# sharonct/CTPA-CLIP

Hardware: AMD Instinct MI355X
Metric: CT-report pairs/sec (contrastive step) (higher is better)
Workload: dtype bf16

## Files before the change

ctpa-clip_amd/csrc/gemm.hip:

```cpp
#include <algorithm>
#include "common.h"
#include "../../include/ctclip_hip.h"

int ctclip_gemm256(const ctclip_gemm_args* a, int split, int batch, void* stream);

namespace {

constexpr int BM = 128, BN = 128, BKT = 64, NTH = 256;
constexpr int KROW = BKT * 2 + 16;
constexpr int TILE_BYTES = 128 * KROW;
constexpr int SMEM_BYTES = 4 * TILE_BYTES;
constexpr int CS_LD = 132;

struct P {
  int64_t M, N, K;
  const u16* A; int64_t lda;
  const u16* B; int64_t ldb;
  const u16* B2;
  void* C; int64_t ldc; int c_f32;
  u16* C2; int64_t ldc2;
  const float* bias;
  const void* R; int64_t ldr; int r_f32;
  float alpha; int act; int accumulate; int split_k;
  int64_t sA, sB, sC, sC2, sR;
// ... 647 lines not shown
    hipLaunchKernelGGL(reduce_slabs_rows_kernel<false>, dim3(blocks), dim3(256), 0, (hipStream_t)stream, slabs, nslab,
                       rows, cols, ld, map, dst, ldd, accumulate);
  CT_CHECK_LAUNCH();
  return 0;
}

extern "C" int ctclip_reduce_slabs(const float* slabs, int64_t nslab, int64_t rows, int64_t cols, int64_t ld,
                                   void* out, int64_t ldo, int32_t out_f32, int32_t accumulate, void* stream) {
  if (rows == 0 || cols == 0) return 0;
  CT_REQUIRE(cols % 4 == 0 && ld % 4 == 0 && ldo % 4 == 0, CT_EALIGN);
  const int64_t total = rows * (cols / 4);
  if (total < 64 * 1024 && nslab >= 16) {
    hipLaunchKernelGGL(reduce_slabs_skinny_kernel, dim3(cdiv(total, 64)), dim3(1024), 0, (hipStream_t)stream, slabs,
                       nslab, rows, cols, ld, out, ldo, out_f32, accumulate);
    CT_CHECK_LAUNCH();
    return 0;
  }
  const int blocks = (int)std::min<int64_t>(4096, (total + 255) / 256);
  hipLaunchKernelGGL(reduce_slabs_kernel, dim3(blocks), dim3(256), 0, (hipStream_t)stream, slabs, nslab, rows, cols,
                     ld, out, ldo, out_f32, accumulate);
  CT_CHECK_LAUNCH();
  return 0;
}
```

ctpa-clip_amd/ctclip_mi355x/_lib.py:

```python
from __future__ import annotations

import ctypes
import os

import torch

_HERE = os.path.dirname(os.path.abspath(__file__))
LIB_PATH = os.environ.get('CTCLIP_HIP_LIB') or os.path.join(_HERE, 'libctclip_hip.so')
_LIB = None

c_i64 = ctypes.c_int64
c_i32 = ctypes.c_int32
c_f32 = ctypes.c_float
c_vp = ctypes.c_void_p


class SlabJob(ctypes.Structure):
    _fields_ = [('slabs', c_vp), ('nslab', c_i64), ('cols', c_i64), ('out', c_vp), ('accumulate', c_i32),
                ('pad', c_i32)]


ABI_VERSION = 2


class GemmArgs(ctypes.Structure):
    _fields_ = [
        ('M', c_i64), ('N', c_i64), ('K', c_i64),
        ('A', c_vp), ('lda', c_i64), ('a_kcontig', c_i32),
        ('B', c_vp), ('ldb', c_i64), ('b_kcontig', c_i32),
        ('C', c_vp), ('ldc', c_i64), ('c_f32', c_i32),
        ('C2', c_vp), ('ldc2', c_i64),
        ('bias', c_vp),
        ('R', c_vp), ('ldr', c_i64), ('r_f32', c_i32),
        ('alpha', c_f32),
        ('act', c_i32),
        ('accumulate', c_i32),
        ('split_k', c_i32),
        ('batch', c_i32),
        ('sA', c_i64), ('sB', c_i64), ('sC', c_i64), ('sC2', c_i64), ('sR', c_i64),
        ('n2', c_i32),
        ('B2', c_vp),
        ('ab_f16', c_i32),
        ('r_f16', c_i32),
# ... 157 lines not shown
    'ctclip_gemm_set_grid_cap': [c_i32],
    'ctclip_reduce_slabs_ep': [c_vp, c_i64, c_i64, c_i64, c_i64, ctypes.POINTER(GemmArgs), c_vp],
    'ctclip_reduce_slabs_ep_drop': [c_vp, c_i64, c_i64, c_i64, c_i64, ctypes.POINTER(GemmArgs), c_f32, ctypes.c_uint64,
                                    c_vp],
    'ctclip_layernorm_bwd_drop': [c_vp, c_i32, c_i64, c_vp, c_i32, c_i64, c_vp, c_vp, c_vp, c_i64, c_i32, c_vp, c_i64,
                                  c_vp, c_i64, c_vp, c_vp, c_vp, c_i32, c_f32, ctypes.c_uint64, c_vp],
    'ctclip_patch_ln_x2': [c_vp, c_i32, c_i32, c_i64, c_i32, c_i32, c_i32, c_i32, c_i32, c_i32, c_vp, c_f32, c_vp,
                           c_vp, c_i64, c_vp],
    'ctclip_patch_ln_x3': [c_vp, c_i32, c_i32, c_i64, c_i32, c_i32, c_i32, c_i32, c_i32, c_i32, c_vp, c_f32, c_vp,
                           c_vp, c_vp, c_i64, c_vp],
    'ctclip_layernorm_fwd_x2': [c_vp, c_i32, c_i64, c_i64, c_i32, c_vp, c_vp, c_f32, c_vp, c_vp, c_i64, c_vp, c_i64,
                                c_vp, c_vp, c_vp],
    'ctclip_layernorm_fwd_x3': [c_vp, c_i32, c_i64, c_i64, c_i32, c_vp, c_vp, c_f32, c_vp, c_vp, c_vp, c_i64, c_vp,
                                c_i64, c_vp, c_vp, c_vp, c_vp],
    'ctclip_pack_rows_h16': [c_vp, c_i64, c_vp, c_i64, c_i32, c_i32, c_vp, c_vp, c_i64, c_vp],
    'ctclip_pack_qkv_fold_h16': [c_vp, c_i64, c_vp, c_i64, c_i64, c_vp, c_i64, c_i64, c_vp, c_i64, c_vp, c_vp],
    'ctclip_skinny_gemm_slices': [c_i64, c_i64, c_i64],
    'ctclip_skinny_gemm': [c_vp, c_i64, c_vp, c_i64, c_i64, c_i64, c_i64, c_vp, c_i32, c_vp],
    'ctclip_vq_l2norm_h16': [c_vp, c_i64, c_i64, c_i32, c_vp, c_i64, c_vp],
    'ctclip_skinny_sgemm_slices': [c_i64, c_i64, c_i64],
    'ctclip_skinny_sgemm': [c_vp, c_i64, c_vp, c_i64, c_i64, c_i64, c_i64, c_vp, c_i32, c_vp],
    'ctclip_reduce_slabs': [c_vp, c_i64, c_i64, c_i64, c_i64, c_vp, c_i64, c_i32, c_i32, c_vp],
    'ctclip_reduce_slabs_multi': [ctypes.POINTER(SlabJob), c_i32, c_vp],
    'ctclip_layernorm_fwd': [c_vp, c_i32, c_i64, c_i64, c_i32, c_vp, c_vp, c_f32, c_vp, c_i64, c_vp, c_i64,
                             c_vp, c_vp, c_vp],
    'ctclip_layernorm_bwd': [c_vp, c_i32, c_i64, c_vp, c_i32, c_i64, c_vp, c_vp, c_vp, c_i64, c_i32, c_vp, c_i64,
                             c_vp, c_i64, c_vp, c_i64, c_vp, c_vp, c_i32, c_vp],
    'ctclip_l2norm_scale_fwd': [c_vp, c_i64, c_i64, c_i32, c_i32, c_vp, c_vp, c_i64, c_vp],
    'ctclip_l2norm_scale_bwd': [c_vp, c_i64, c_vp, c_i64, c_i64, c_i32, c_i32, c_vp, c_vp, c_i64, c_vp, c_i32, c_vp],
    'ctclip_l2norm_scale_bwd_fold': [c_vp, c_i64, c_vp, c_i64, c_i64, c_i32, c_i32, c_vp, c_vp, c_i64, c_vp, c_i32,
                                     c_vp, c_vp, c_vp, c_i64, c_vp, c_vp, c_i32, c_vp, c_vp, c_vp],
    'ctclip_colsum': [c_vp, c_i32, c_i64, c_i64, c_i32, c_vp, c_i32, c_vp],
    'ctclip_geglu_bwd': [c_vp, c_i64, c_vp, c_i64, c_i64, c_i32, c_vp, c_i64, c_vp],
    'ctclip_gelu_bwd': [c_vp, c_vp, c_vp, c_i64, c_vp],
    'ctclip_pack_rows': [c_vp, c_i64, c_vp, c_i64, c_i32, c_i32, c_vp, c_vp, c_i64, c_vp],
    'ctclip_pack_rows_f32': [c_vp, c_i64, c_vp, c_i64, c_i32, c_i32, c_vp, c_vp, c_i64, c_vp],
    'ctclip_split_f16': [c_vp, c_i64, c_i64, c_i32, c_f32, c_vp, c_vp, c_i64, c_vp, c_vp],
    'ctclip_pack_rows_x3': [c_vp, c_i64, c_vp, c_i64, c_i32, c_i32, c_vp, c_f32, c_vp, c_vp, c_i64, c_vp, c_vp],
    'ctclip_sgemm_tn': [ctypes.POINTER(SgemmTnArgs), c_vp],
    'ctclip_unpack_rows': [c_vp, c_i64, c_vp, c_i64, c_i32, c_vp, c_i64, c_i32, c_vp],
    'ctclip_reduce_slabs_rows': [c_vp, c_i64, c_i64, c_i64, c_i64, c_vp, c_vp, c_i64, c_i32, c_vp],
    'ctclip_gelu_f32': [c_vp, c_vp, c_i64, c_vp],
    'ctclip_cast_f32_bf16': [c_vp, c_vp, c_i64, c_vp],
    'ctclip_cast_f32_bf16_split': [c_vp, c_vp, c_vp, c_i64, c_vp],
    'ctclip_add_f32': [c_vp, c_vp, c_vp, c_vp, c_i64, c_vp],
    'ctclip_patch_ln': [c_vp, c_i32, c_i32, c_i64, c_i32, c_i32, c_i32, c_i32, c_i32, c_i32, c_vp, c_f32, c_vp, c_i64,
# ... 128 lines not shown
```

ctpa-clip_amd/ctclip_mi355x/functional.py:

```python
from __future__ import annotations

import math
import os
import weakref
from dataclasses import dataclass

import torch

from . import dist_sync
from . import kernels as K
from . import streams

F32, BF16 = torch.float32, torch.bfloat16


def gsink(p):
    if not p.requires_grad:
        return None
    if p.grad is None:
        p.grad = torch.zeros_like(p, memory_format=torch.contiguous_format)
    return p.grad


def gsink_cat(ps):
# ... 521 lines not shown
            x3f = K.linear(g, W2p, residual=x2f, out_dtype=F32, out2=x3b)
        else:
            h = K.linear(xn2, W1p, act=K.ACT_GEGLU, out2=g, tag='ff1',
                         flops=2.0 * xf.shape[0] * W1.shape[0] * W1.shape[1])
            x3f = K.linear(g, W2p, residual=x2f, out_dtype=F32, out2=x3b)
        if lean:
            ctx.mark_non_differentiable(x3b)
            return x3f, x3b
        ctx.geo = geo
        ctx.use_bias = use_bias
        ctx.fold = fold
        ctx.fold_w = (Wp, cs) if fold else None
        ctx.params = (peg_w, peg_b, norm_g, q_scale, k_scale, Wq, Wkv, Wo, ff_w, ff_b, W1, W2)
        ctx.save_for_backward(xb, x1b, m1, r1, xn, q, kv, qn, kn, o, lse, x2b, m2, r2, xn2, h, g,
                              bias_u if use_bias else torch.empty(0), Wq_b, Wkv_b, Wo_b, W1p, W2p)
        ctx.mark_non_differentiable(x3b)
        ctx.set_materialize_grads(False)
        return x3f, x3b

    @staticmethod
    def backward(ctx, dx3f, _dx3b):
        if dx3f is None:
            return (None,) * 16
        (xb, x1b, m1, r1, xn, q, kv, qn, kn, o, lse, x2b, m2, r2, xn2, h, g, bias_u, Wq_b, Wkv_b, Wo_b, W1p,
         W2p) = ctx.saved_tensors
        peg_w, peg_b, norm_g, q_scale, k_scale, Wq, Wkv, Wo, ff_w, ff_b, W1, W2 = ctx.params
        geo = ctx.geo
        H, dh = geo.heads, geo.dim_head
        inner = H * dh
        dev = dx3f.device
        dx3b = take_shadow(dx3f)
        dx3f = dx3f.contiguous()
        if dx3b is None:
            dx3b = K.cast_bf16(dx3f)
        dh_ = K.matmul_nn_geglu_bwd(dx3b, W2p, h)
        M_ = dx3b.shape[0]
        if gsink(W2) is not None:
            K.matmul_tn(dx3b, g, tag='dw', flops=2.0 * M_ * W2.shape[0] * W2.shape[1],
                        unpack=(gsink(W2), None, W2.shape[1]))
        fused = K.matmul_nn_ln_bwd(dh_, W1p, x2b, m2, r2, ff_w, dx3f, dgamma_out=gsink(ff_w),
                                   dbeta_out=gsink(ff_b)) if K.ln_guarded() else None
        if fused is None:
            dxn2 = K.matmul_nn(dh_, W1p)
        if gsink(W1) is not None:
            rmap = ff1_rowmap(W1.shape[0] // 2, dev)
            K.matmul_tn(dh_, xn2, tag='dw', flops=2.0 * M_ * W1.shape[0] * W1.shape[1],
                        unpack=(gsink(W1), rmap, W1.shape[1]))
        if fused is not None:
            dx2f, dx2b = fused
        else:
            dx2f, dx2b, _, _ = K.layernorm_bwd(dxn2, x2b, m2, r2, ff_w, dres=dx3f, dgamma_out=gsink(ff_w),
                                               dbeta_out=gsink(ff_b))
        do = K.matmul_nn(dx2b, Wo_b)
        K.matmul_tn(dx2b, o, out=gsink(Wo), accumulate=True, tag='dw')
        dqn = torch.empty_like(qn)
        dkn = torch.empty_like(kn)
        L, nseq, seq = geo.seq()
        du = None
        if ctx.use_bias:
            acc = ctx.bias_acc
            if acc['du'] is None:
                acc['du'] = torch.zeros_like(bias_u)
            du = acc['du']
        fold = getattr(ctx, 'fold', False)
        if fold:
            Wp, cs = ctx.fold_w
            M_ = qn.shape[0]
            dqkv = torch.empty(M_, 3 * inner, device=dev, dtype=BF16)
            dqkn = torch.empty(M_, 2 * inner, device=dev, dtype=BF16)
            K.attn_bwd(qn, kn, kv[:, inner:], o, lse, do, dqkn[:, :inner], dqkn[:, inner:], dqkv[:, 2 * inner:],
                       L=L, H=H, D=dh, nseq=nseq, scale=8.0, seq=seq, bias_u=bias_u if ctx.use_bias else None,
                       dbias_u=du, grid=(geo.Hg, geo.Wg) if ctx.use_bias else (0, 0))
            _bias_grad_ready(ctx, du)
            qk = q.as_strided((M_, 2 * inner), q.stride())
            _, _, u1, c1, be1 = K.l2norm_qk_bwd_fold(qk, dqkn, q_scale, k_scale, r1, m1, dqkv[:, :2 * inner], cs,
                                                     x1b.shape[1], ds_q_out=gsink(q_scale),
                                                     ds_k_out=gsink(k_scale))
            Gqkv = K.matmul_tn(dqkv, x1b, tag='dw')
            gq, gkv = gsink(Wq), gsink(Wkv)
            K.lnfold_wgrad(Gqkv, u1, norm_g, gq if gq is not None else torch.empty(Wq.shape, device=dev),
                           wq=Wq.detach(), grad_gamma=gsink(norm_g),
                           grad_rest=gkv if gkv is not None else torch.empty(Wkv.shape, device=dev))
            dx1f, dx1b = K.matmul_lnfold_bwd(dqkv, Wp, dx2f, x1b, c1, be1)
        else:
            dkv = torch.empty_like(kv)
            K.attn_bwd(qn, kn, kv[:, inner:], o, lse, do, dqn, dkn, dkv[:, inner:], L=L, H=H, D=dh, nseq=nseq,
                       scale=8.0, seq=seq, bias_u=bias_u if ctx.use_bias else None, dbias_u=du,
                       grid=(geo.Hg, geo.Wg) if ctx.use_bias else (0, 0))
            _bias_grad_ready(ctx, du)
            dq = torch.empty(q.shape, device=dev, dtype=q.dtype)
            K.l2norm_scale_bwd(q, dqn, H, dh, q_scale, dq, ds_out=gsink(q_scale))
            K.l2norm_scale_bwd(kv[:, :inner], dkn, H, dh, k_scale, dkv[:, :inner], ds_out=gsink(k_scale))
            fusable = K.ln_guarded() and K.ln_fusable(dq.shape[0], Wq_b.shape[1], bwd=True)
            if not fusable:
                dxn = K.matmul_nn(dq, Wq_b)
            K.matmul_tn(dq, xn, out=gsink(Wq), accumulate=True, tag='dw')
            K.matmul_tn(dkv, x1b, out=gsink(Wkv), accumulate=True, tag='dw')
            dx1kv = K.matmul_nn(dkv, Wkv_b, residual=dx2f, out_dtype=F32)
            fused = K.matmul_nn_ln_bwd(dq, Wq_b, x1b, m1, r1, norm_g, dx1kv, dgamma_out=gsink(norm_g)) \
                if fusable else None
            if fused is not None:
                dx1f, dx1b = fused
            else:
                if fusable:
                    dxn = K.matmul_nn(dq, Wq_b)
                dx1f, dx1b, _, _ = K.layernorm_bwd(dxn, x1b, m1, r1, norm_g, dres=dx1kv, want_beta=False,
                                                   dgamma_out=gsink(norm_g))
        dxf, dxb, _, _ = K.peg_bwd(dx1b, dx1f, xb, geo.B, geo.T, geo.Hg, geo.Wg, peg_w, geo.mode,
                                   dweight_out=gsink(peg_w), dbias_out=gsink(peg_b))
        put_shadow(dxf, dxb)
        if du is not None:
            if ctx.bias_first:
                ctx.bias_acc['du'] = None
            else:
                du = None
        return (dxf, None, du, None, None, None, None, None, None, None, None, None, None,
                None, None, None)


def _fold_shape_ok(geo, dim, Wkv):
# ... 596 lines not shown
```

ctpa-clip_amd/ctclip_mi355x/kernels.py:

```python
from __future__ import annotations

import contextlib
import os

import torch

from . import _lib
from ._lib import GemmArgs, LnEpilogueArgs, call, ptr, stream_ptr

BF16 = torch.bfloat16
F32 = torch.float32
F16 = torch.float16

ACT_NONE, ACT_GELU, ACT_GEGLU, ACT_ARGMAX, ACT_GEGLU_BWD, ACT_L2N, ACT_GELU_BWD = 0, 1, 2, 3, 4, 5, 6


def _chk(t, name, dtype=None):
    if not t.is_cuda:
        raise ValueError(f'{name}: expected a device tensor')
    if dtype is not None and t.dtype != dtype:
        raise ValueError(f'{name}: expected {dtype}, got {t.dtype}')


class KernelTimer:
# ... 276 lines not shown
    reduce_param_partials(pg, dgamma_out, True)
    if dbeta_out is not None:
        reduce_param_partials(pb, dbeta_out, True)
    return dxf, dxb


def matmul_nn_gelu_bwd(dy, w, pre, out=None):
    M, N = dy.shape
    K = w.shape[1]
    assert w.shape[0] == N and pre.shape == (M, K) and pre.dtype == BF16
    if out is None:
        out = torch.empty(M, K, device=dy.device, dtype=BF16)
    gemm_raw(M, K, N, dy, dy.stride(0), True, w, w.stride(0), False, out, out.stride(0), R=pre, ldr=pre.stride(0),
             act=ACT_GELU_BWD)
    return out


def split_for(m_rows, tiles):
    target = 512
    s = max(1, min(target // max(tiles, 1), m_rows // 1024))
    return max(1, s)


def matmul_tn(dy, x, *, out=None, accumulate=False, split_k=None, alpha=1.0, tag=None, flops=None, unpack=None):
    M, N = dy.shape
    K = x.shape[1]
    assert x.shape[0] == M
    if out is None:
        out = torch.zeros(N, K, device=dy.device, dtype=F32) if accumulate else \
            torch.empty(N, K, device=dy.device, dtype=F32)
    if split_k is not None:
        s = split_k
    elif N >= 256 and K >= 256 and M % 64 == 0 and M >= 64 * 1024:
        t256 = ((N + 255) // 256) * ((K + 255) // 256)
        s = max(1, 256 // t256)
        if t256 * s < 160:
            s = split_for(M, ((N + 127) // 128) * ((K + 127) // 128))
    else:
        s = split_for(M, ((N + 127) // 128) * ((K + 127) // 128))
    if s <= 1:
        gemm_raw(N, K, M, dy, dy.stride(0), False, x, x.stride(0), False, out, out.stride(0),
                 accumulate=accumulate, alpha=alpha, tag=tag, flops=flops)
        if unpack is not None:
            dst, rowmap, cols = unpack
            return unpack_rows(out, dst, rowmap=rowmap, cols=cols, accumulate=True)
        return out
    slabs = torch.empty(s, N, K, device=dy.device, dtype=F32)
    gemm_raw(N, K, M, dy, dy.stride(0), False, x, x.stride(0), False, slabs, K, split_k=s, alpha=alpha, tag=tag,
             flops=flops)
    if unpack is not None:
        dst, rowmap, cols = unpack
        assert dst.dtype == F32 and dst.stride(1) == 1 and cols <= K
        assert rowmap is None or (rowmap.dtype == torch.int32 and rowmap.numel() == N)
        call('ctclip_reduce_slabs_rows', ptr(slabs), s, N, cols, K, ptr(rowmap), ptr(dst), dst.stride(0), 1,
             stream_ptr())
        return dst
    reduce_slabs(slabs, out, accumulate=accumulate)
    return out


def reduce_slabs(slabs, out, accumulate=False):
    s, rows, cols = slabs.shape
    call('ctclip_reduce_slabs', ptr(slabs), s, rows, cols, cols, ptr(out), out.stride(0),
         int(out.dtype == F32), int(accumulate), stream_ptr())
    return out


_DEFERRED = {}
_CB_QUEUED = [None]


def _graph_task():
    try:
        return torch._C._current_graph_task_id()
    except AttributeError:
        return -1


def _in_backward():
    return _graph_task() != -1


def discard_deferred():
    _DEFERRED.clear()
    _CB_QUEUED[0] = None


def flush_reductions(lo=None, hi=None):
    used = []
    for k in list(_DEFERRED):
        st, jobs = _DEFERRED[k]
        if lo is None:
            take, keep = jobs, []
        else:
            take = [j for j in jobs if lo <= j[1].data_ptr() < hi]
            keep = [j for j in jobs if not (lo <= j[1].data_ptr() < hi)]
        if keep:
            _DEFERRED[k] = (st, keep)
        else:
            del _DEFERRED[k]
        if not take:
            continue
        while take:
            seen, batch, rest = set(), [], []
            for j in take:
                (rest if j[1].data_ptr() in seen else batch).append(j)
                seen.add(j[1].data_ptr())
            arr = (_lib.SlabJob * len(batch))()
            for i, (sl, out, acc) in enumerate(batch):
                arr[i].slabs, arr[i].nslab, arr[i].cols = sl.data_ptr(), sl.shape[0], sl.shape[-1]
                arr[i].out, arr[i].accumulate = out.data_ptr(), int(acc)
            call('ctclip_reduce_slabs_multi', arr, len(batch), st.cuda_stream)
            take = rest
        used.append(st)
    return used


def _end_of_backward():
    _CB_QUEUED[0] = None
    flush_reductions()


def reduce_param_partials(part, out, accumulate):
    nb, D = part.shape[0], part.shape[-1]
    if (nb >= 16 and out.dtype == F32 and out.is_contiguous() and part.is_contiguous()
            and D % 4 == 0 and _in_backward()):
        st = torch.cuda.current_stream(part.device)
        _DEFERRED.setdefault(st.cuda_stream, (st, []))[1].append((part, out.view(-1), accumulate))
        task = _graph_task()
        if _CB_QUEUED[0] != task:
            torch.autograd.Variable._execution_engine.queue_callback(_end_of_backward)
            _CB_QUEUED[0] = task
        return out
    return reduce_slabs(part.view(nb, 1, D), out.view(1, D), accumulate=accumulate)


def nblocks_for(rows, cap=1024):
    return int(max(1, min(cap, max((rows + 63) // 64, min(256, (rows + 3) // 4)))))


def colsum(x, out=None, accumulate=False):
    rows, cols = x.shape
    nb = int(max(1, min(256, rows // 8)))
    part = torch.empty(nb, cols, device=x.device, dtype=F32)
    call('ctclip_colsum', ptr(x), int(x.dtype == F32), x.stride(0), rows, cols, ptr(part), nb, stream_ptr())
    if out is None:
        out = torch.zeros(cols, device=x.device, dtype=F32) if accumulate else torch.empty(cols, device=x.device,
                                                                                           dtype=F32)
    if accumulate:
        reduce_param_partials(part, out, accumulate)
    else:
        reduce_slabs(part.view(nb, 1, cols), out.view(1, cols), accumulate=accumulate)
    return out


# ... 325 lines not shown
    reduce_slabs(part_u.view(nb, 1, H * D), u.view(1, H * D))
    if ds_out is not None:
        ds = reduce_param_partials(part, ds_out, True)
    else:
        ds = torch.empty(D, device=x.device, dtype=F32)
        reduce_slabs(part.view(nb, 1, D), ds.view(1, D))
    return ds, dx2, u, c1, beta


def l2norm_qk_bwd_fold(qk, dqk, q_scale, k_scale, row_rstd, row_mean, out, fold_cs, Dm, ds_q_out=None,
                       ds_k_out=None):
    rows = qk.shape[0]
    assert qk.shape[1] == 512 and dqk.shape[1] == 512 and out.shape[1] == 512
    nb = 1024
    dev = qk.device
    part_s = torch.empty(2, nb, 32, device=dev, dtype=F32)
    part_u = torch.empty(nb, 256, device=dev, dtype=F32)
    c1 = torch.empty(rows, device=dev, dtype=F32)
    beta = torch.empty(rows, device=dev, dtype=F32)
    call('ctclip_l2norm_qk_bwd_fold', ptr(qk), qk.stride(0), ptr(dqk), dqk.stride(0), rows, ptr(q_scale),
         ptr(k_scale), ptr(out), out.stride(0), ptr(part_s), nb, ptr(row_rstd), ptr(row_mean), ptr(part_u),
         ptr(fold_cs), int(Dm), ptr(c1), ptr(beta), stream_ptr())
    u = torch.empty(256, device=dev, dtype=F32)
    reduce_slabs(part_u.view(nb, 1, 256), u.view(1, 256))
    ds = []
    for i, sink in ((0, ds_q_out), (1, ds_k_out)):
        if sink is not None:
            ds.append(reduce_param_partials(part_s[i], sink, True))
        else:
            d = torch.empty(32, device=dev, dtype=F32)
            reduce_slabs(part_s[i].view(nb, 1, 32), d.view(1, 32))
            ds.append(d)
    return ds[0], ds[1], u, c1, beta


def lnfold_wgrad(G, u, gamma, grad_q, *, wq=None, grad_gamma=None, grad_rest=None):
    nq = grad_q.shape[0]
    Kd = G.shape[1]
    nrest = G.shape[0] - nq
    assert nrest == 0 or grad_rest is not None
    g = gamma.detach().contiguous()
    call('ctclip_lnfold_wgrad', ptr(G), G.stride(0), ptr(u), ptr(g), ptr(wq), wq.stride(0) if wq is not None else 0,
         nq, nrest, Kd, ptr(grad_q), grad_q.stride(0), ptr(grad_gamma), ptr(grad_rest),
         grad_rest.stride(0) if grad_rest is not None else 0, stream_ptr())
    return grad_q


def matmul_lnfold_bwd(dqkv, wp, res, x, c1, beta, out=None, out2=None):
    M, Kq = dqkv.shape
    N = wp.shape[1]
    assert wp.shape[0] == Kq and dqkv.stride(1) == 1 and wp.stride(1) == 1
    if out is None:
        out = torch.empty(M, N, device=dqkv.device, dtype=F32)
    if out2 is None:
        out2 = torch.empty(M, N, device=dqkv.device, dtype=BF16)
    assert out.dtype == F32 and res.dtype == F32
    a = _gemm_args(M, N, Kq, dqkv, wp, out, b_kcontig=False, C2=out2, R=res)
    call('ctclip_gemm_lnfold_bwd', _lib.ctypes.byref(a), ptr(x), x.stride(0), ptr(c1), ptr(beta), stream_ptr())
    return out, out2


def peg_bwd(doutb, doutf, xb, B, T, H, W, weight, mode, dweight_out=None, dbias_out=None):
    D = xb.shape[1]
    dxf = torch.empty_like(doutf)
    dxb = torch.empty_like(doutb)
    rc = _CT_ESHAPE
    if _PEG_BWD_X32 and doutf.is_contiguous():
        rc = _lib.lib().ctclip_peg_bwd_data_x32(ptr(doutf), B, T, H, W, D, ptr(weight), mode, ptr(dxf), ptr(dxb),
                                                stream_ptr())
    if rc == _CT_ESHAPE:
        call('ctclip_peg_bwd_data', ptr(doutb), ptr(doutf), B, T, H, W, D, ptr(weight), mode, ptr(dxf), ptr(dxb),
             stream_ptr())
    elif rc != 0:
        raise _lib.KernelError(f'ctclip_peg_bwd_data_x32 failed with code {rc}')
    nblk = _lib.lib().ctclip_peg_wgrad_slabs(B, T, H, W, D)
    part = torch.empty(nblk, D * 28, device=xb.device, dtype=F32)
    call('ctclip_peg_bwd_weight', ptr(doutb), ptr(xb), B, T, H, W, D, mode, ptr(part), nblk, stream_ptr())
    if dweight_out is not None or dbias_out is not None:
        assert dweight_out is None or (dweight_out.is_contiguous() and dweight_out.numel() == D * 27)
        assert dbias_out is None or (dbias_out.is_contiguous() and dbias_out.numel() == D)
        call('ctclip_peg_wgrad_reduce', ptr(part), nblk, D, ptr(dweight_out), ptr(dbias_out), 1, stream_ptr())
        return dxf, dxb, dweight_out, dbias_out
    dw = torch.empty(D, 27, device=xb.device, dtype=F32)
    db = torch.empty(D, device=xb.device, dtype=F32)
    call('ctclip_peg_wgrad_reduce', ptr(part), nblk, D, ptr(dw), ptr(db), 0, stream_ptr())
    return dxf, dxb, dw, db


def _attn_args(q, k, v, o, *, L, H, D, nseq, M, scale, seq, bias_u=None, grid=(0, 0), kmask=None, lse=None,
               dout=None, dq=None, dk=None, dv=None, delta=None, dbias_u=None, dropout=(0.0, 0)):
    a = _lib.AttnArgs()
    a.q, a.ldq = ptr(q), q.stride(0)
    a.k, a.ldk = ptr(k), k.stride(0)
    a.v, a.ldv = ptr(v), v.stride(0)
    a.o, a.ldo = ptr(o), o.stride(0)
    a.dout, a.lddo = ptr(dout), dout.stride(0) if dout is not None else 0
    a.dq, a.lddq = ptr(dq), dq.stride(0) if dq is not None else 0
    a.dk, a.lddk = ptr(dk), dk.stride(0) if dk is not None else 0
    a.dv, a.lddv = ptr(dv), dv.stride(0) if dv is not None else 0
    a.lse, a.delta = ptr(lse), ptr(delta)
    a.bias_u, a.dbias_u, a.kmask = ptr(bias_u), ptr(dbias_u), ptr(kmask)
    a.scale, a.L, a.H, a.D, a.nseq, a.M = scale, L, H, D, nseq, M
    a.grid_h, a.grid_w = grid
# ... 769 lines not shown
```

ctpa-clip_amd/ctclip_mi355x/trainer.py:

```python
from __future__ import annotations

import collections
import os
from types import SimpleNamespace as _Rows

import torch


from . import checkpoint
from . import dist_sync
from . import streams
from . import kernels as K


def _ema_site():
    from . import ct_clip
    return ct_clip.DEFER_EMA


STATUS_COPY_STREAM = os.environ.get('CTCLIP_STATUS_COPY_STREAM', '1') != '0'


class FlatParams:

# ... 508 lines not shown
                if TEXT_FIRST:
                    back_img()
        finally:
            model.defer_text_backward = False
            model.set_ema_mode(old)

    def _train_step_chunked(self, text, video, chunk):
        from . import functional as Fn
        self._check_ln(block_upto=self.steps - 2)
        model = self.model
        keep = None
        if self.keep_chunk_latents:
            keep = {'pass2_text': [], 'pass2_image': [], 'indices': []}
        self.grad_sync.arm()
        dist_sync.disarm()
        try:
            with K.ln_guard():
                tc, ic, states = self._chunked_pass1(text, video, chunk)
                loss, dt, di, dlt = Fn.clip_loss_all_rows(tc, ic, model.temperature,
                                                          bool(model.decoupled_contrastive_learning))
                if model.temperature.requires_grad:
                    self.flat.rebind_grads([model.temperature])
                    model.temperature.grad.add_(dlt.reshape(()))
                self._chunked_pass2(text, video, chunk, dt, di, states, keep)
            model.apply_held_ema()
        except BaseException:
            dist_sync.disarm()
            K.discard_deferred()
            model._deferred_text = model._deferred_image = None
            model.drop_held_ema()
            streams.flush_text(self.device)
            streams.join_text(self.device)
            streams.join_aux(self.device)
            self.flat.grad.zero_()
            raise
        self.last_chunked = dict(text_cache=tc, image_cache=ic, dropout_states=states, **(keep or {}))
        self.optimizer_step()
        self._queue_ln_check()
        return loss.detach()
```

include/ctclip_hip.h:

```cpp
#ifndef CTCLIP_HIP_H
#define CTCLIP_HIP_H
#include <stdint.h>
#ifdef __cplusplus
extern "C" {
#endif

#define CTCLIP_ABI_VERSION 2
#define CT_STATUS_LN_TIMEOUT 1
#define CT_STATUS_F16_RANGE 2
#define CT_STATUS_NONFINITE_GRAD 4
#define CT_STATUS_VQ_NONFINITE 8
int ctclip_version(void);
int ctclip_device_arch(char* buf, int n);
int ctclip_debug_hold_cus(int32_t nwg, int64_t cycles, int32_t lds_bytes, void* stream);

typedef struct {
  int64_t M, N, K;
  const void* A; int64_t lda; int32_t a_kcontig;
  const void* B; int64_t ldb; int32_t b_kcontig;
  void* C; int64_t ldc; int32_t c_f32;
  void* C2; int64_t ldc2;
  const float* bias;
  const void* R; int64_t ldr; int32_t r_f32;
  float alpha;
// ... 56 lines not shown
int ctclip_gemm_lnfold_bwd(const ctclip_gemm_args* a, const void* X, int64_t ldx, const float* c1, const float* beta,
                           void* stream);
int ctclip_lnfold_wgrad(const float* G, int64_t ldg, const float* u, const float* gamma, const float* Wq, int64_t ldw,
                        int64_t nq, int64_t nrest, int64_t K, float* grad_q, int64_t ldgq, float* grad_gamma,
                        float* grad_rest, int64_t ldgr, void* stream);

int ctclip_skinny_gemm_slices(int64_t M, int64_t N, int64_t K);
int ctclip_skinny_gemm(const void* A, int64_t lda, const void* B, int64_t ldb, int64_t M, int64_t N, int64_t K,
                       float* slabs, int32_t nslices, void* stream);
int ctclip_skinny_sgemm_slices(int64_t M, int64_t N, int64_t K);
int ctclip_skinny_sgemm(const float* A, int64_t lda, const float* B, int64_t ldb, int64_t M, int64_t N, int64_t K,
                        float* slabs, int32_t nslices, void* stream);
int ctclip_reduce_slabs_rows(const float* slabs, int64_t nslab, int64_t rows, int64_t cols, int64_t ld,
                             const int32_t* map, float* dst, int64_t ldd, int32_t accumulate, void* stream);
int ctclip_reduce_slabs(const float* slabs, int64_t nslab, int64_t rows, int64_t cols, int64_t ld,
                        void* out, int64_t ldo, int32_t out_f32, int32_t accumulate, void* stream);
typedef struct {
  const float* slabs;
  int64_t nslab, cols;
  float* out;
  int32_t accumulate, pad;
} ctclip_slab_job;
int ctclip_reduce_slabs_multi(const ctclip_slab_job* jobs, int32_t njobs, void* stream);
int ctclip_reduce_slabs_ep(const float* slabs, int64_t nslab, int64_t rows, int64_t cols, int64_t ld,
                           const ctclip_gemm_args* ep, void* stream);


typedef struct {
  int64_t M, N, Kp;
  const void* A; int64_t lda; const void* sA;
  const void* B; int64_t ldb; const void* sB;
  void* C; int64_t ldc; int32_t c_f32;
  const float* bias; float alpha;
  const float* R; int64_t ldr;
  void* C2; int64_t ldc2;
  int32_t act;
} ctclip_mx_gemm_args;
int ctclip_quant_mxfp8(const void* x, int32_t x_f32, int64_t rows, int64_t K, int64_t ldx, void* q, int64_t ldq,
                       void* scales, int64_t Kp, void* stream);
int ctclip_gemm_mxfp8(const ctclip_mx_gemm_args* a, void* stream);
int ctclip_gemm_mxfp8_set_tile(int bm);

int ctclip_layernorm_fwd_x2(const void* x, int32_t x_f32, int64_t ldx, int64_t rows, int32_t D, const float* gamma,
                            const float* beta, float eps, void* y_bf16, void* y_f16, int64_t ldyb, float* y_f32,
                            int64_t ldyf, float* mean, float* rstd, void* stream);
int ctclip_layernorm_fwd_x3(const void* x, int32_t x_f32, int64_t ldx, int64_t rows, int32_t D, const float* gamma,
// ... 326 lines not shown
```

Measured before the change: 208.4.

## Batch per-layer weight-gradient slab reductions into one grouped finish kernel

Weight-gradient epilogues in the ViT layer backward (split-K slab sums, skinny reductions, LN-fold weight/gamma grads, PEG wgrad) are now queued as jobs instead of being launched one by one. At the end of each layer's backward they are grouped into a single job-table kernel launch, with dependency levels computed from pointer-range overlaps. The aim is fewer small kernel launches and better GPU fill from running independent reductions concurrently. It adds host-side bookkeeping and is disabled during the chunked second pass.

```diff
diff --git a/ctpa-clip_amd/csrc/gemm.hip b/ctpa-clip_amd/csrc/gemm.hip
--- a/ctpa-clip_amd/csrc/gemm.hip
+++ b/ctpa-clip_amd/csrc/gemm.hip
@@ -1,4 +1,5 @@
 #include <algorithm>
+#include <vector>
 #include "common.h"
 #include "../../include/ctclip_hip.h"
 
@@ -693,3 +694,222 @@
   CT_CHECK_LAUNCH();
   return 0;
 }
+
+constexpr int FIN_JOBS = 16;
+constexpr int64_t FIN_CHUNK = 16384;
+constexpr int FIN_MAX_BLOCKS = 4096;
+struct FinTable {
+  ctclip_finish_job j[FIN_JOBS];
+  int32_t blk0[FIN_JOBS + 1];
+  int32_t v4[FIN_JOBS];
+  int32_t n;
+};
+
+template <bool V4>
+__device__ __forceinline__ void fin_sum(const ctclip_finish_job& jb, int64_t b, int64_t nb) {
+  constexpr int W = V4 ? 4 : 1;
+  const float* __restrict__ s = jb.src;
+  const int64_t rows = jb.rows, ld = jb.ld, nw = jb.cols / W, total = rows * nw;
+  for (int64_t i = b * 256 + threadIdx.x; i < total; i += nb * 256) {
+    const int64_t r = i / nw, c = (i - r * nw) * W;
+    const int64_t dr = jb.map ? (int64_t)jb.map[r] : r;
+    if (dr < 0 || dr >= jb.dst_rows) continue;
+    if constexpr (V4) {
+      f32x4 acc = {0.f, 0.f, 0.f, 0.f};
+      for (int64_t z = 0; z < jb.nslab; ++z) acc += *(const f32x4*)(s + (z * rows + r) * ld + c);
+      f32x4* o = (f32x4*)(jb.dst + dr * jb.ldd + c);
+      *o = jb.accumulate ? *o + acc : acc;
+    } else {
+      float acc = 0.f;
+      for (int64_t z = 0; z < jb.nslab; ++z) acc += s[(z * rows + r) * ld + c];
+      float* o = jb.dst + dr * jb.ldd + c;
+      *o = jb.accumulate ? *o + acc : acc;
+    }
+  }
+}
+
+__global__ __launch_bounds__(256) void grad_finish_kernel(FinTable t) {
+  __shared__ f32x4 red[16][16];
+  int ji = 0;
+  while (ji + 1 < t.n && (int)blockIdx.x >= t.blk0[ji + 1]) ++ji;
+  const ctclip_finish_job jb = t.j[ji];
+  const int64_t b = (int)blockIdx.x - t.blk0[ji], nb = t.blk0[ji + 1] - t.blk0[ji];
+  const int tid = threadIdx.x;
+  if (jb.kind == CT_FIN_SUM) {
+    if (t.v4[ji]) fin_sum<true>(jb, b, nb);
+    else fin_sum<false>(jb, b, nb);
+  } else if (jb.kind == CT_FIN_SKINNY) {
+    const int c4 = tid & 15, lane = tid >> 4;
+    const int64_t n4 = jb.cols / 4, total = jb.rows * n4;
+    for (int64_t g = b; g * 16 < total; g += nb) {
+      const int64_t e = g * 16 + c4;
+      const bool valid = e < total;
+      const int64_t r = valid ? e / n4 : 0, c = valid ? (e - r * n4) * 4 : 0;
+      f32x4 acc = {0.f, 0.f, 0.f, 0.f};
+      if (valid) {
+#pragma unroll 4
+        for (int64_t z = lane; z < jb.nslab; z += 16) acc += *(const f32x4*)(jb.src + (z * jb.rows + r) * jb.ld + c);
+      }
+      red[lane][c4] = acc;
+      __syncthreads();
+      if (lane == 0 && valid) {
+        for (int k = 1; k < 16; ++k) acc += red[k][c4];
+        float* o = jb.dst + r * jb.ldd + c;
+        if (jb.accumulate) acc += *(const f32x4*)o;
+        *(f32x4*)o = acc;
+      }
+      __syncthreads();
+    }
+  } else if (jb.kind == CT_FIN_LNFOLD_W) {
+    const float* __restrict__ G = jb.src;
+    const int64_t K = jb.cols, nq = jb.rows, total = (nq + jb.nrest) * K;
+    for (int64_t i = b * 256 + tid; i < total; i += nb * 256) {
+      const int64_t n = i / K, k = i - n * K;
+      if (n < nq) jb.dst[n * jb.ldd + k] += jb.gamma[k] * (G[n * jb.ld + k] - jb.u[n]);
+      else jb.dst2[(n - nq) * jb.ldd2 + k] += G[n * jb.ld + k];
+    }
+  } else if (jb.kind == CT_FIN_LNFOLD_G) {
+    float* part = (float*)red;
+    const float* __restrict__ G = jb.src;
+    const int lane = tid & 63, w = tid >> 6;
+    const int64_t K = jb.cols, nq = jb.rows;
+    for (int64_t g = b; g * 64 < K; g += nb) {
+      const int64_t k = g * 64 + lane;
+      float s = 0.f;
+      if (k < K) {
+#pragma unroll 8
+        for (int64_t n = w; n < nq; n += 4) s = fmaf(jb.wq[n * jb.ldw + k], G[n * jb.ld + k] - jb.u[n], s);
+      }
+      part[w * 64 + lane] = s;
+      __syncthreads();
+      if (w == 0 && k < K) jb.dst[k] += ((part[lane] + part[64 + lane]) + part[128 + lane]) + part[192 + lane];
+      __syncthreads();
+    }
+  } else {
+    const int64_t total = jb.cols * 28;
+    for (int64_t i = b * 256 + tid; i < total; i += nb * 256) {
+      float s = 0.f;
+#pragma unroll 8
+      for (int64_t z = 0; z < jb.nslab; ++z) s += jb.src[z * total + i];
+      const int64_t c = i / 28, k = i - c * 28;
+      float* o = k < 27 ? (jb.dst ? jb.dst + c * 27 + k : nullptr) : (jb.dst2 ? jb.dst2 + c : nullptr);
+      if (o) *o = jb.accumulate ? *o + s : s;
+    }
+  }
+}
+
+namespace {
+struct FinRange {
+  const char *lo, *hi;
+};
+inline FinRange fin_range(const float* p, int64_t floats) {
+  return {(const char*)p, (const char*)(p + (p ? floats : 0))};
+}
+inline bool fin_overlap(const FinRange& a, const FinRange& b) { return a.lo < b.hi && b.lo < a.hi; }
+struct FinInfo {
+  int64_t units, bytes;
+  bool v4;
+  FinRange w[2], r[2];
+  int level, blocks;
+};
+
+int fin_describe(const ctclip_finish_job& j, FinInfo& f) {
+  f = FinInfo{};
+  CT_REQUIRE(j.src && (j.dst || (j.kind == CT_FIN_PEG && j.dst2)) && j.nslab >= 0 && j.rows >= 0 && j.cols >= 0 &&
+                 j.cols <= j.ld,
+             CT_EINVAL);
+  switch (j.kind) {
+    case CT_FIN_SUM: {
+      CT_REQUIRE(j.dst_rows >= 0 && j.cols <= j.ldd && (j.map || j.dst_rows >= j.rows), CT_EINVAL);
+      f.v4 = j.cols % 4 == 0 && j.ld % 4 == 0 && j.ldd % 4 == 0 && aligned16(j.src) && aligned16(j.dst);
+      f.units = cdiv(j.rows * (f.v4 ? j.cols / 4 : j.cols), 256);
+      f.bytes = j.nslab * j.rows * j.cols * 4;
+      f.w[0] = fin_range(j.dst, j.dst_rows ? (j.dst_rows - 1) * j.ldd + j.cols : 0);
+      f.r[0] = fin_range(j.src, j.nslab * j.rows * j.ld);
+      break;
+    }
+    case CT_FIN_SKINNY:
+      CT_REQUIRE(j.cols <= j.ldd, CT_EINVAL);
+      CT_REQUIRE(j.cols % 4 == 0 && j.ld % 4 == 0 && j.ldd % 4 == 0 && aligned16(j.src) && aligned16(j.dst), CT_EALIGN);
+      f.units = cdiv(j.rows * (j.cols / 4), 16);
+      f.bytes = j.nslab * j.rows * j.cols * 4;
+      f.w[0] = fin_range(j.dst, j.rows ? (j.rows - 1) * j.ldd + j.cols : 0);
+      f.r[0] = fin_range(j.src, j.nslab * j.rows * j.ld);
+      break;
+    case CT_FIN_LNFOLD_W:
+      CT_REQUIRE(j.u && j.gamma && j.nrest >= 0 && j.cols <= j.ldd && (j.nrest == 0 || (j.dst2 && j.cols <= j.ldd2)),
+                 CT_EINVAL);
+      f.units = cdiv((j.rows + j.nrest) * j.cols, 256);
+      f.bytes = (j.rows + j.nrest) * j.cols * 12;
+      f.w[0] = fin_range(j.dst, j.rows ? (j.rows - 1) * j.ldd + j.cols : 0);
+      f.w[1] = fin_range(j.dst2, j.nrest ? (j.nrest - 1) * j.ldd2 + j.cols : 0);
+      f.r[0] = fin_range(j.src, (j.rows + j.nrest) * j.ld);
+      f.r[1] = fin_range(j.u, j.rows);
+      break;
+    case CT_FIN_LNFOLD_G:
+      CT_REQUIRE(j.u && j.wq && j.cols <= j.ldw, CT_EINVAL);
+      f.units = cdiv(j.cols, 64);
+      f.bytes = j.rows * j.cols * 8;
+      f.w[0] = fin_range(j.dst, j.cols);
+      f.r[0] = fin_range(j.src, j.rows * j.ld);
+      f.r[1] = fin_range(j.u, j.rows);
+      break;
+    case CT_FIN_PEG:
+      f.units = cdiv(j.cols * 28, 256);
+      f.bytes = j.nslab * j.cols * 28 * 4;
+      f.w[0] = fin_range(j.dst, j.cols * 27);
+      f.w[1] = fin_range(j.dst2, j.cols);
+      f.r[0] = fin_range(j.src, j.nslab * j.cols * 28);
+      break;
+    default:
+      return CT_EINVAL;
+  }
+  f.blocks = (int)std::min<int64_t>(std::min<int64_t>(f.units, FIN_MAX_BLOCKS), std::max<int64_t>(1, cdiv(f.bytes, FIN_CHUNK)));
+  return 0;
+}
+}
+
+extern "C" int ctclip_grad_finish(const ctclip_finish_job* jobs, int32_t njobs, void* stream) {
+  if (njobs <= 0) return 0;
+  CT_REQUIRE(jobs, CT_EINVAL);
+  std::vector<FinInfo> info(njobs);
+  int levels = 0;
+  for (int32_t i = 0; i < njobs; ++i) {
+    const int rc = fin_describe(jobs[i], info[i]);
+    if (rc) return rc;
+    int lv = 0;
+    for (int32_t k = 0; k < i; ++k) {
+      bool dep = false;
+      for (int a = 0; a < 2 && !dep; ++a)
+        for (int c = 0; c < 2 && !dep; ++c)
+          dep = fin_overlap(info[k].w[a], info[i].w[c]) || fin_overlap(info[k].w[a], info[i].r[c]) ||
+                fin_overlap(info[k].r[a], info[i].w[c]);
+      if (dep) lv = std::max(lv, info[k].level + 1);
+    }
+    info[i].level = lv;
+    levels = std::max(levels, lv + 1);
+  }
+  for (int lv = 0; lv < levels; ++lv) {
+    std::vector<int32_t> ids;
+    for (int32_t i = 0; i < njobs; ++i)
+      if (info[i].level == lv && info[i].blocks > 0) ids.push_back(i);
+    std::stable_sort(ids.begin(), ids.end(), [&](int32_t a, int32_t b) {
+      return info[a].bytes / info[a].blocks > info[b].bytes / info[b].blocks;
+    });
+    for (size_t i0 = 0; i0 < ids.size(); i0 += FIN_JOBS) {
+      FinTable t{};
+      t.n = (int32_t)std::min<size_t>(FIN_JOBS, ids.size() - i0);
+      int32_t grid = 0;
+      for (int32_t i = 0; i < t.n; ++i) {
+        t.j[i] = jobs[ids[i0 + i]];
+        t.v4[i] = info[ids[i0 + i]].v4;
+        t.blk0[i] = grid;
+        grid += info[ids[i0 + i]].blocks;
+      }
+      for (int32_t i = t.n; i <= FIN_JOBS; ++i) t.blk0[i] = grid;
+      hipLaunchKernelGGL(grad_finish_kernel, dim3(grid), dim3(256), 0, (hipStream_t)stream, t);
+      CT_CHECK_LAUNCH();
+    }
+  }
+  return 0;
+}
diff --git a/ctpa-clip_amd/ctclip_mi355x/_lib.py b/ctpa-clip_amd/ctclip_mi355x/_lib.py
--- a/ctpa-clip_amd/ctclip_mi355x/_lib.py
+++ b/ctpa-clip_amd/ctclip_mi355x/_lib.py
@@ -19,6 +19,16 @@
     _fields_ = [('slabs', c_vp), ('nslab', c_i64), ('cols', c_i64), ('out', c_vp), ('accumulate', c_i32),
                 ('pad', c_i32)]
 
+
+class FinishJob(ctypes.Structure):
+    _fields_ = [('kind', c_i32), ('accumulate', c_i32), ('src', c_vp),
+                ('nslab', c_i64), ('rows', c_i64), ('cols', c_i64), ('ld', c_i64),
+                ('map', c_vp), ('dst', c_vp), ('ldd', c_i64), ('dst_rows', c_i64),
+                ('u', c_vp), ('gamma', c_vp), ('wq', c_vp), ('ldw', c_i64),
+                ('dst2', c_vp), ('ldd2', c_i64), ('nrest', c_i64)]
+
+
+FIN_SUM, FIN_SKINNY, FIN_LNFOLD_W, FIN_LNFOLD_G, FIN_PEG = range(5)
 
 ABI_VERSION = 2
 
@@ -222,6 +232,7 @@
     'ctclip_skinny_sgemm': [c_vp, c_i64, c_vp, c_i64, c_i64, c_i64, c_i64, c_vp, c_i32, c_vp],
     'ctclip_reduce_slabs': [c_vp, c_i64, c_i64, c_i64, c_i64, c_vp, c_i64, c_i32, c_i32, c_vp],
     'ctclip_reduce_slabs_multi': [ctypes.POINTER(SlabJob), c_i32, c_vp],
+    'ctclip_grad_finish': [ctypes.POINTER(FinishJob), c_i32, c_vp],
     'ctclip_layernorm_fwd': [c_vp, c_i32, c_i64, c_i64, c_i32, c_vp, c_vp, c_f32, c_vp, c_i64, c_vp, c_i64,
                              c_vp, c_vp, c_vp],
     'ctclip_layernorm_bwd': [c_vp, c_i32, c_i64, c_vp, c_i32, c_i64, c_vp, c_vp, c_vp, c_i64, c_i32, c_vp, c_i64,
diff --git a/ctpa-clip_amd/ctclip_mi355x/functional.py b/ctpa-clip_amd/ctclip_mi355x/functional.py
--- a/ctpa-clip_amd/ctclip_mi355x/functional.py
+++ b/ctpa-clip_amd/ctclip_mi355x/functional.py
@@ -567,6 +567,11 @@
     def backward(ctx, dx3f, _dx3b):
         if dx3f is None:
             return (None,) * 16
+        with K.grad_finisher():
+            return ViTLayerFn._backward(ctx, dx3f)
+
+    @staticmethod
+    def _backward(ctx, dx3f):
         (xb, x1b, m1, r1, xn, q, kv, qn, kn, o, lse, x2b, m2, r2, xn2, h, g, bias_u, Wq_b, Wkv_b, Wo_b, W1p,
          W2p) = ctx.saved_tensors
         peg_w, peg_b, norm_g, q_scale, k_scale, Wq, Wkv, Wo, ff_w, ff_b, W1, W2 = ctx.params
@@ -582,7 +587,7 @@
         M_ = dx3b.shape[0]
         if gsink(W2) is not None:
             K.matmul_tn(dx3b, g, tag='dw', flops=2.0 * M_ * W2.shape[0] * W2.shape[1],
-                        unpack=(gsink(W2), None, W2.shape[1]))
+                        unpack=(gsink(W2), None, W2.shape[1]), finish=True)
         fused = K.matmul_nn_ln_bwd(dh_, W1p, x2b, m2, r2, ff_w, dx3f, dgamma_out=gsink(ff_w),
                                    dbeta_out=gsink(ff_b)) if K.ln_guarded() else None
         if fused is None:
@@ -590,14 +595,14 @@
         if gsink(W1) is not None:
             rmap = ff1_rowmap(W1.shape[0] // 2, dev)
             K.matmul_tn(dh_, xn2, tag='dw', flops=2.0 * M_ * W1.shape[0] * W1.shape[1],
-                        unpack=(gsink(W1), rmap, W1.shape[1]))
+                        unpack=(gsink(W1), rmap, W1.shape[1]), finish=True)
         if fused is not None:
             dx2f, dx2b = fused
         else:
             dx2f, dx2b, _, _ = K.layernorm_bwd(dxn2, x2b, m2, r2, ff_w, dres=dx3f, dgamma_out=gsink(ff_w),
                                                dbeta_out=gsink(ff_b))
         do = K.matmul_nn(dx2b, Wo_b)
-        K.matmul_tn(dx2b, o, out=gsink(Wo), accumulate=True, tag='dw')
+        K.matmul_tn(dx2b, o, out=gsink(Wo), accumulate=True, tag='dw', finish=True)
         dqn = torch.empty_like(qn)
         dkn = torch.empty_like(kn)
         L, nseq, seq = geo.seq()
@@ -621,7 +626,7 @@
             _, _, u1, c1, be1 = K.l2norm_qk_bwd_fold(qk, dqkn, q_scale, k_scale, r1, m1, dqkv[:, :2 * inner], cs,
                                                      x1b.shape[1], ds_q_out=gsink(q_scale),
                                                      ds_k_out=gsink(k_scale))
-            Gqkv = K.matmul_tn(dqkv, x1b, tag='dw')
+            Gqkv = K.matmul_tn(dqkv, x1b, tag='dw', finish=True)
             gq, gkv = gsink(Wq), gsink(Wkv)
             K.lnfold_wgrad(Gqkv, u1, norm_g, gq if gq is not None else torch.empty(Wq.shape, device=dev),
                            wq=Wq.detach(), grad_gamma=gsink(norm_g),
@@ -639,8 +644,8 @@
             fusable = K.ln_guarded() and K.ln_fusable(dq.shape[0], Wq_b.shape[1], bwd=True)
             if not fusable:
                 dxn = K.matmul_nn(dq, Wq_b)
-            K.matmul_tn(dq, xn, out=gsink(Wq), accumulate=True, tag='dw')
-            K.matmul_tn(dkv, x1b, out=gsink(Wkv), accumulate=True, tag='dw')
+            K.matmul_tn(dq, xn, out=gsink(Wq), accumulate=True, tag='dw', finish=True)
+            K.matmul_tn(dkv, x1b, out=gsink(Wkv), accumulate=True, tag='dw', finish=True)
             dx1kv = K.matmul_nn(dkv, Wkv_b, residual=dx2f, out_dtype=F32)
             fused = K.matmul_nn_ln_bwd(dq, Wq_b, x1b, m1, r1, norm_g, dx1kv, dgamma_out=gsink(norm_g)) \
                 if fusable else None
diff --git a/ctpa-clip_amd/ctclip_mi355x/kernels.py b/ctpa-clip_amd/ctclip_mi355x/kernels.py
--- a/ctpa-clip_amd/ctclip_mi355x/kernels.py
+++ b/ctpa-clip_amd/ctclip_mi355x/kernels.py
@@ -322,7 +322,8 @@
     return max(1, s)
 
 
-def matmul_tn(dy, x, *, out=None, accumulate=False, split_k=None, alpha=1.0, tag=None, flops=None, unpack=None):
+def matmul_tn(dy, x, *, out=None, accumulate=False, split_k=None, alpha=1.0, tag=None, flops=None, unpack=None,
+              finish=False):
     M, N = dy.shape
     K = x.shape[1]
     assert x.shape[0] == M
@@ -352,15 +353,25 @@
         dst, rowmap, cols = unpack
         assert dst.dtype == F32 and dst.stride(1) == 1 and cols <= K
         assert rowmap is None or (rowmap.dtype == torch.int32 and rowmap.numel() == N)
+        if finish and _FINISH[0]:
+            _queue_finish(_lib.FIN_SUM, (slabs, rowmap), (dst,), accumulate=1, src=ptr(slabs), nslab=s, rows=N,
+                          cols=cols, ld=K, map=ptr(rowmap), dst=ptr(dst), ldd=dst.stride(0), dst_rows=dst.shape[0])
+            return dst
         call('ctclip_reduce_slabs_rows', ptr(slabs), s, N, cols, K, ptr(rowmap), ptr(dst), dst.stride(0), 1,
              stream_ptr())
         return dst
-    reduce_slabs(slabs, out, accumulate=accumulate)
-    return out
-
-
-def reduce_slabs(slabs, out, accumulate=False):
+    reduce_slabs(slabs, out, accumulate=accumulate, finish=finish)
+    return out
+
+
+def reduce_slabs(slabs, out, accumulate=False, finish=False):
     s, rows, cols = slabs.shape
+    if finish and _FINISH[0] and out.dtype == F32 and rows * cols:
+        skinny = rows * (cols // 4) < 64 * 1024 and s >= 16
+        _queue_finish(_lib.FIN_SKINNY if skinny else _lib.FIN_SUM, (slabs,), (out,), accumulate=int(accumulate),
+                      src=ptr(slabs), nslab=s, rows=rows, cols=cols, ld=cols, dst=ptr(out), ldd=out.stride(0),
+                      dst_rows=rows)
+        return out
     call('ctclip_reduce_slabs', ptr(slabs), s, rows, cols, cols, ptr(out), out.stride(0),
          int(out.dtype == F32), int(accumulate), stream_ptr())
     return out
@@ -368,6 +379,74 @@
 
 _DEFERRED = {}
 _CB_QUEUED = [None]
+GRAD_FINISH = True
+_FINISH = [False]
+
+
+class FinishJob:
+    __slots__ = ('fields', 'keep', 'outs')
+
+    def __init__(self, fields, keep, outs):
+        self.fields, self.keep, self.outs = fields, keep, [o for o in outs if o is not None]
+
+
+def _job_in(j, lo, hi):
+    outs = j.outs if isinstance(j, FinishJob) else (j[1],)
+    return any(lo <= o.data_ptr() < hi for o in outs)
+
+
+def _queue_job(job, device=None):
+    st = torch.cuda.current_stream(device)
+    _DEFERRED.setdefault(st.cuda_stream, (st, []))[1].append(job)
+    task = _graph_task()
+    if _CB_QUEUED[0] != task:
+        torch.autograd.Variable._execution_engine.queue_callback(_end_of_backward)
+        _CB_QUEUED[0] = task
+
+
+def _queue_finish(kind, keep, outs, **fields):
+    _queue_job(FinishJob(dict(fields, kind=kind), keep, outs), outs[0].device)
+
+
+def _launch_finish(st, jobs):
+    arr = (_lib.FinishJob * len(jobs))()
+    for a, j in zip(arr, jobs):
+        for k, v in j.fields.items():
+            setattr(a, k, v)
+    call('ctclip_grad_finish', arr, len(jobs), st.cuda_stream)
+
+
+@contextlib.contextmanager
+def grad_finisher():
+    if not (GRAD_FINISH and _in_backward()) or _FINISH[0]:
+        yield
+        return
+    _FINISH[0] = True
+    try:
+        yield
+    finally:
+        _FINISH[0] = False
+    key = torch.cuda.current_stream().cuda_stream
+    if key in _DEFERRED:
+        st, jobs = _DEFERRED[key]
+        mine = [j for j in jobs if isinstance(j, FinishJob)]
+        rest = [j for j in jobs if not isinstance(j, FinishJob)]
+        if rest:
+            _DEFERRED[key] = (st, rest)
+        else:
+            del _DEFERRED[key]
+        if mine:
+            _launch_finish(st, mine)
+
+
+@contextlib.contextmanager
+def grad_finish_off():
+    global GRAD_FINISH
+    was, GRAD_FINISH = GRAD_FINISH, False
+    try:
+        yield
+    finally:
+        GRAD_FINISH = was
 
 
 def _graph_task():
@@ -393,14 +472,18 @@
         if lo is None:
             take, keep = jobs, []
         else:
-            take = [j for j in jobs if lo <= j[1].data_ptr() < hi]
-            keep = [j for j in jobs if not (lo <= j[1].data_ptr() < hi)]
+            take = [j for j in jobs if _job_in(j, lo, hi)]
+            keep = [j for j in jobs if not _job_in(j, lo, hi)]
         if keep:
             _DEFERRED[k] = (st, keep)
         else:
             del _DEFERRED[k]
         if not take:
             continue
+        fin = [j for j in take if isinstance(j, FinishJob)]
+        if fin:
+            _launch_finish(st, fin)
+            take = [j for j in take if not isinstance(j, FinishJob)]
         while take:
             seen, batch, rest = set(), [], []
             for j in take:
@@ -425,12 +508,7 @@
     nb, D = part.shape[0], part.shape[-1]
     if (nb >= 16 and out.dtype == F32 and out.is_contiguous() and part.is_contiguous()
             and D % 4 == 0 and _in_backward()):
-        st = torch.cuda.current_stream(part.device)
-        _DEFERRED.setdefault(st.cuda_stream, (st, []))[1].append((part, out.view(-1), accumulate))
-        task = _graph_task()
-        if _CB_QUEUED[0] != task:
-            torch.autograd.Variable._execution_engine.queue_callback(_end_of_backward)
-            _CB_QUEUED[0] = task
+        _queue_job((part, out.view(-1), accumulate), part.device)
         return out
     return reduce_slabs(part.view(nb, 1, D), out.view(1, D), accumulate=accumulate)
 
@@ -802,7 +880,7 @@
          ptr(k_scale), ptr(out), out.stride(0), ptr(part_s), nb, ptr(row_rstd), ptr(row_mean), ptr(part_u),
          ptr(fold_cs), int(Dm), ptr(c1), ptr(beta), stream_ptr())
     u = torch.empty(256, device=dev, dtype=F32)
-    reduce_slabs(part_u.view(nb, 1, 256), u.view(1, 256))
+    reduce_slabs(part_u.view(nb, 1, 256), u.view(1, 256), finish=True)
     ds = []
     for i, sink in ((0, ds_q_out), (1, ds_k_out)):
         if sink is not None:
@@ -820,6 +898,15 @@
     nrest = G.shape[0] - nq
     assert nrest == 0 or grad_rest is not None
     g = gamma.detach().contiguous()
+    if _FINISH[0]:
+        common = dict(src=ptr(G), ld=G.stride(0), rows=nq, cols=Kd, u=ptr(u))
+        _queue_finish(_lib.FIN_LNFOLD_W, (G, u, g), (grad_q, grad_rest), gamma=ptr(g), nrest=nrest, dst=ptr(grad_q),
+                      ldd=grad_q.stride(0), dst2=ptr(grad_rest),
+                      ldd2=grad_rest.stride(0) if grad_rest is not None else 0, **common)
+        if grad_gamma is not None:
+            _queue_finish(_lib.FIN_LNFOLD_G, (G, u, wq), (grad_gamma,), wq=ptr(wq), ldw=wq.stride(0),
+                          dst=ptr(grad_gamma), **common)
+        return grad_q
     call('ctclip_lnfold_wgrad', ptr(G), G.stride(0), ptr(u), ptr(g), ptr(wq), wq.stride(0) if wq is not None else 0,
          nq, nrest, Kd, ptr(grad_q), grad_q.stride(0), ptr(grad_gamma), ptr(grad_rest),
          grad_rest.stride(0) if grad_rest is not None else 0, stream_ptr())
@@ -859,6 +946,11 @@
     if dweight_out is not None or dbias_out is not None:
         assert dweight_out is None or (dweight_out.is_contiguous() and dweight_out.numel() == D * 27)
         assert dbias_out is None or (dbias_out.is_contiguous() and dbias_out.numel() == D)
+        if _FINISH[0]:
+            _queue_finish(_lib.FIN_PEG, (part,), [o for o in (dweight_out, dbias_out) if o is not None],
+                          accumulate=1, src=ptr(part), nslab=nblk, cols=D, ld=D, dst=ptr(dweight_out),
+                          dst2=ptr(dbias_out))
+            return dxf, dxb, dweight_out, dbias_out
         call('ctclip_peg_wgrad_reduce', ptr(part), nblk, D, ptr(dweight_out), ptr(dbias_out), 1, stream_ptr())
         return dxf, dxb, dweight_out, dbias_out
     dw = torch.empty(D, 27, device=xb.device, dtype=F32)
diff --git a/ctpa-clip_amd/ctclip_mi355x/trainer.py b/ctpa-clip_amd/ctclip_mi355x/trainer.py
--- a/ctpa-clip_amd/ctclip_mi355x/trainer.py
+++ b/ctpa-clip_amd/ctclip_mi355x/trainer.py
@@ -554,7 +554,8 @@
                 if model.temperature.requires_grad:
                     self.flat.rebind_grads([model.temperature])
                     model.temperature.grad.add_(dlt.reshape(()))
-                self._chunked_pass2(text, video, chunk, dt, di, states, keep)
+                with K.grad_finish_off():
+                    self._chunked_pass2(text, video, chunk, dt, di, states, keep)
             model.apply_held_ema()
         except BaseException:
             dist_sync.disarm()
diff --git a/include/ctclip_hip.h b/include/ctclip_hip.h
--- a/include/ctclip_hip.h
+++ b/include/ctclip_hip.h
@@ -102,6 +102,26 @@
   int32_t accumulate, pad;
 } ctclip_slab_job;
 int ctclip_reduce_slabs_multi(const ctclip_slab_job* jobs, int32_t njobs, void* stream);
+#define CT_FIN_SUM 0
+#define CT_FIN_SKINNY 1
+#define CT_FIN_LNFOLD_W 2
+#define CT_FIN_LNFOLD_G 3
+#define CT_FIN_PEG 4
+typedef struct {
+  int32_t kind, accumulate;
+  const float* src;
+  int64_t nslab, rows, cols, ld;
+  const int32_t* map;
+  float* dst;
+  int64_t ldd, dst_rows;
+  const float* u;
+  const float* gamma;
+  const float* wq;
+  int64_t ldw;
+  float* dst2;
+  int64_t ldd2, nrest;
+} ctclip_finish_job;
+int ctclip_grad_finish(const ctclip_finish_job* jobs, int32_t njobs, void* stream);
 int ctclip_reduce_slabs_ep(const float* slabs, int64_t nslab, int64_t rows, int64_t cols, int64_t ld,
                            const ctclip_gemm_args* ep, void* stream);
 
```

New measurement: 208.4, median of 2. No clear change (+0.0%).
